# l-johnson-code/glTF-Renderer

Measured on AMD Instinct MI355X. Metric: Mrays/sec + ms/frame @1920x1080, 8-bounce, 1/2/4/8 MI355X, higher is better.
Workload: dtype f32

## Files before the change

### gltf_renderer_amd/csrc/pt_debug_kernels.h

```cpp
#include "pt_vertex.h"
#include "pt_host.h"

namespace pt {
namespace {

__global__ __launch_bounds__(kBlock) void k_debug_sample_texture(SceneRec sc, const uint32_t* __restrict__ mat_slot, const float* __restrict__ tc,
                                                              uint32_t n, float* __restrict__ out, int32_t* __restrict__ taps) {
    stage_luts(sc);
    stage_materials(sc);
    const uint32_t i = blockIdx.x * kBlock + threadIdx.x;
    if (i >= n) return;
    const vec2 uv[2] = {{tc[4 * i], tc[4 * i + 1]}, {tc[4 * i + 2], tc[4 * i + 3]}};
    int32_t t5[5];
    const vec4 r = debug_sample_query(sc, mat_slot[2 * i], (int)mat_slot[2 * i + 1], uv, t5);
    out[4 * i] = r.x; out[4 * i + 1] = r.y; out[4 * i + 2] = r.z; out[4 * i + 3] = r.w;
    for (int c = 0; c < 5; c++) taps[5 * i + c] = t5[c];
}
void launch_debug_sample_texture(const SceneRec& sc, const uint32_t* d_mat_slot, const float* d_tc, uint32_t n, float* d_out, int32_t* d_taps, hipStream_t stream) {
    if (n == 0) return;
    hipLaunchKernelGGL(k_debug_sample_texture, dim3((n + kBlock - 1) / kBlock), dim3(kBlock), 0, stream, sc, d_mat_slot, d_tc, n, d_out, d_taps);
}
__global__ __launch_bounds__(kBlock) void k_debug_env_query(SceneRec sc, int op, const float* __restrict__ in, uint32_t n, float* __restrict__ out) {
#ifdef PT_LUT_LDS
    __shared__ int s_stack[kStackLds * kBlock];
    static_assert((size_t)kStackLds * kBlock * sizeof(int) >= (size_t)kImpLdsFloat4 * sizeof(float4), "the traversal stack's LDS must hold the importance pyramid's coarse levels");
    float4* top = (float4*)s_stack;
    stage_importance_top_into(sc, top);
#else
    const float4* top = importance_lds_top();
#endif
    const uint32_t i = blockIdx.x * kBlock + threadIdx.x;
    if (i >= n) return;
    debug_env_query(sc, op, in + (size_t)kEnvQueryIn * i, out + (size_t)kEnvQueryOut * i, top);
}
void launch_debug_env_query(const SceneRec& sc, int op, const float* d_in, uint32_t n, float* d_out, hipStream_t stream) {
    if (n == 0) return;
    hipLaunchKernelGGL(k_debug_env_query, dim3((n + kBlock - 1) / kBlock), dim3(kBlock), 0, stream, sc, op, d_in, n, d_out);
}
__global__ __launch_bounds__(kBlock) void k_debug_bsdf_query(SceneRec sc, int op, uint32_t flags, const float* __restrict__ in, uint32_t n, float* __restrict__ out) {
    stage_luts(sc);
    const uint32_t i = blockIdx.x * kBlock + threadIdx.x;
    if (i >= n) return;
    debug_bsdf_query(sc, op, flags, in + (size_t)kBsdfQueryIn * i, out + (size_t)kBsdfQueryOut * i);
}
void launch_debug_bsdf_query(const SceneRec& sc, int op, uint32_t flags, const float* d_in, uint32_t n, float* d_out, hipStream_t stream) {
    if (n == 0) return;
    hipLaunchKernelGGL(k_debug_bsdf_query, dim3((n + kBlock - 1) / kBlock), dim3(kBlock), 0, stream, sc, op, flags, d_in, n, d_out);
}
__global__ __launch_bounds__(kBlock) void k_debug_light_query(SceneRec sc_in, uint32_t small_tables, int num_of_lights, const uint32_t* __restrict__ index,
                                                           const float* __restrict__ p, uint32_t n, float* __restrict__ out) {
    SceneRec sc = sc_in; sc.small_tables = small_tables ? 1u : 0u;
    stage_lights(sc, num_of_lights);
    const uint32_t i = blockIdx.x * kBlock + threadIdx.x;
    if (i >= n) return;
    debug_light_query(sc, index[i], v3(p[3 * (size_t)i], p[3 * (size_t)i + 1], p[3 * (size_t)i + 2]), out + (size_t)kLightQueryOut * i);
}
void launch_debug_light_query(const SceneRec& sc, bool small_tables, int num_of_lights, const uint32_t* d_index, const float* d_p, uint32_t n, float* d_out, hipStream_t stream) {
    if (n == 0) return;
    hipLaunchKernelGGL(k_debug_light_query, dim3((n + kBlock - 1) / kBlock), dim3(kBlock), 0, stream, sc, small_tables ? 1u : 0u, num_of_lights, d_index, d_p, n, d_out);
}
__global__ __launch_bounds__(kBlock) void k_debug_surface_query(SceneRec sc_in, uint32_t small_tables, uint32_t flags, const float* __restrict__ in, uint32_t n, float* __restrict__ out) {
    SceneRec sc = sc_in; sc.small_tables = small_tables ? 1u : 0u;
    stage_luts(sc);
    stage_tangent_lut(sc);
    stage_instances(sc);
    stage_materials(sc);
    const uint32_t i = blockIdx.x * kBlock + threadIdx.x;
    if (i >= n) return;
    debug_surface_query(sc, flags, in + (size_t)kSurfQueryIn * i, out + (size_t)kSurfQueryOut * i);
}
void launch_debug_surface_query(const SceneRec& sc, bool small_tables, uint32_t flags, const float* d_in, uint32_t n, float* d_out, hipStream_t stream) {
    if (n == 0) return;
    hipLaunchKernelGGL(k_debug_surface_query, dim3((n + kBlock - 1) / kBlock), dim3(kBlock), 0, stream, sc, small_tables ? 1u : 0u, flags, d_in, n, d_out);
}
constexpr DebugQueryLaunch kDebugQueryLaunch = {launch_debug_sample_texture, launch_debug_env_query, launch_debug_bsdf_query, launch_debug_light_query, launch_debug_surface_query};

// ... 3 lines not shown
```

### gltf_renderer_amd/csrc/pt_shading.h

```cpp
#pragma once
#include "pt_math.h"
#include "pt_types.h"

namespace pt {

constexpr float kMinRoughness = 0.001f;

PT_DEV vec4 next_random(uint32_t px, uint32_t py, uint32_t seed, int& count) {
    uint32_t x = px * 1664525u + 1013904223u, y = py * 1664525u + 1013904223u;
    uint32_t z = seed * 1664525u + 1013904223u, w = (uint32_t)count * 1664525u + 1013904223u;
    count++;
    x += y * w; y += z * x; z += x * y; w += y * z;
    x ^= x >> 16; y ^= y >> 16; z ^= z >> 16; w ^= w >> 16;
    x += y * w; y += z * x; z += x * y; w += y * z;
    const float s = 2.3283064365386963e-10f;
    return {(float)x * s, (float)y * s, (float)z * s, (float)w * s};
}

PT_DEV vec3 decode_octahedral(float ex, float ey) {
    float z = 1.f - fabsf(ex) - fabsf(ey);
    float x = ex, y = ey;
    if (!(z >= 0.f)) {
        x = (ex >= 0 ? 1.f : -1.f) * (1.f - fabsf(ey));
        y = (ey >= 0 ? 1.f : -1.f) * (1.f - fabsf(ex));
// ... 274 lines not shown
    vec3 n, t;
    float tw;
    if (has_ts) {
        vec3 n0, n1, n2, t0, t1, t2;
        float w0, w1, w2;
        decode_tangent_space(ts0, tangent_sincos(sc, (ts0 >> 20) & 0x3ffu), n0, t0, w0);
        decode_tangent_space(ts1, tangent_sincos(sc, (ts1 >> 20) & 0x3ffu), n1, t1, w1);
        decode_tangent_space(ts2, tangent_sincos(sc, (ts2 >> 20) & 0x3ffu), n2, t2, w2);
        n = w.x * n0 + w.y * n1 + w.z * n2;
        t = w.x * t0 + w.y * t1 + w.z * t2;
        tw = w0;
    } else {
        n = ng;
        vec3 helper = v3(1, 0, 0);
        if (fabsf(ng.x) > fabsf(ng.y)) helper = v3(0, 1, 0);
        t = normalize(cross(helper, ng));
        tw = 1;
    }
    a.position = mul_point(in.T, pos);
    a.ng = normalize(mul_dir(in.N, ng));
    a.n = normalize(mul_dir(in.N, n));
    a.t = normalize(mul_dir(in.T, t));
    a.tw = tw;
    a.bt = tw * normalize(cross(a.n, a.t));
    return a;
}

struct Surface {
    vec3 albedo; float alpha, metalness, ax, ay;
    vec3 n, at, ab; float ior;
    vec3 spec_color; float spec_factor, clearcoat, cc_rough;
    vec3 cc_n, sheen_color; float sheen_a, transmissive;
    vec3 emissive_texel;
    float sheen_lh, sheen_sv;
};
struct MatHeader {
    uint32_t flags; int32_t alpha_mode; float metalness_factor, roughness_factor;
    vec4 base_color_factor;
    vec3 emissive_factor; float alpha_cutoff;
    float ior, normal_scale, specular_factor, clearcoat_normal_scale;
    vec3 specular_color_factor; float clearcoat_factor;
    float clearcoat_roughness_factor, anisotropy_strength, anisotropy_cos, anisotropy_sin;
    vec3 sheen_color_factor; float sheen_roughness_factor;
    float transmission_factor; uint32_t bound_mask;
    const uint4* trio;
};
PT_DEV MatHeader load_mat_header(const RMat* m) {
    const float4* q = (const float4*)m;
    const float4 a = q[0], b = q[1], c = q[2], d = q[3], e = q[4], f = q[5], g = q[6], h = q[7];
    MatHeader r;
    r.flags = __float_as_uint(a.x); r.alpha_mode = __float_as_int(a.y); r.metalness_factor = a.z; r.roughness_factor = a.w;
    r.base_color_factor = {b.x, b.y, b.z, b.w};
    r.emissive_factor = v3(c.x, c.y, c.z); r.alpha_cutoff = c.w;
    r.ior = d.x; r.normal_scale = d.y; r.specular_factor = d.z; r.clearcoat_normal_scale = d.w;
    r.specular_color_factor = v3(e.x, e.y, e.z); r.clearcoat_factor = e.w;
    r.clearcoat_roughness_factor = f.x; r.anisotropy_strength = f.y; r.anisotropy_cos = f.z; r.anisotropy_sin = f.w;
    r.sheen_color_factor = v3(g.x, g.y, g.z); r.sheen_roughness_factor = g.w;
    r.transmission_factor = h.x; r.bound_mask = __float_as_uint(h.y);
    r.trio = (const uint4*)(((uint64_t)__float_as_uint(h.w) << 32) | (uint64_t)__float_as_uint(h.z));
    return r;
}
PT_DEV bool slot_bound(uint32_t mask, int slot) { return (mask >> slot) & 1u; }
#ifdef PT_LUT_LDS
constexpr uint32_t kMatCacheMax = 96;
constexpr uint32_t kMatCacheRecs = 17;
static __shared__ float4 pt_lds_mat[kMatCacheMax * kMatCacheRecs];
PT_DEV bool materials_cached(const SceneRec& sc) { return sc.small_tables || sc.n_materials <= kMatCacheMax; }
// ... 182 lines not shown
        const PbrTexels f = fetch_pbr_texels(sc, mid, h, tc);
        const int s = slot == 16 ? SLOT_ALBEDO : slot == 17 ? SLOT_NORMAL : slot == 18 ? SLOT_METALLIC_ROUGHNESS : SLOT_EMISSIVE;
        const bool trio = (h.bound_mask & RM_TRIO) != 0;
        const RTex t = load_rtex(&m->tex[trio ? SLOT_ALBEDO : s]);
        base = t.texels;
        if (slot == 16) { k = f.k_alb; r = resolve_taps(k, f.a00, f.a10, f.a01, f.a11, sc.srgb_lut); }
        else if (slot == 17) { k = f.k_nrm; r = resolve_taps(k, f.n00, f.n10, f.n01, f.n11, sc.srgb_lut); }
        else if (slot == 18) { k = f.k_mr; r = resolve_taps(k, f.m00, f.m10, f.m01, f.m11, sc.srgb_lut); }
        else if (trio && (h.bound_mask & RM_TRIO_EMISSIVE)) { k = f.k_alb; r = f.emissive; }
        else { const RTex te = load_rtex(&m->tex[SLOT_EMISSIVE]); k = texture_taps(te, tc); base = te.texels; r = sample_slot(sc, m, SLOT_EMISSIVE, tc, taps); }
    }
    taps5[0] = k.i0; taps5[1] = k.i1;
    taps5[2] = (int32_t)((k.p0 - base) / k.width); taps5[3] = (int32_t)((k.p1 - base) / k.width);
    taps5[4] = k.ia;
    return r;
}

PT_DEV float schlick(float f0, float c) { return f0 + (1 - f0) * hpow5(1 - fabsf(c)); }
PT_DEV vec3 schlick3(vec3 f0, float c) { return f0 + (1 - f0) * hpow5(1 - fabsf(c)); }
PT_DEV float ggx_d(float a, float ndh) {
    float a2 = a * a;
    float den = ndh * ndh * (a2 - 1) + 1;
    den *= kPi * den;
    return fdiv(a2 * heavyside(ndh), den);
}
PT_DEV float ggx_corr_v(float a, float ndl, float ndv, float hdl, float hdv) {
    float a2 = a * a;
    float num = 0.5f * heavyside(hdl) * heavyside(hdv);
    float den = fabsf(ndv) * sqrtf(a2 + (1 - a2) * ndl * ndl);
    den += fabsf(ndl) * sqrtf(a2 + (1 - a2) * ndv * ndv);
    return fdiv(num, den);
}
PT_DEV float specular_brdf(float a, float ndl, float ndv, float ndh, float hdl, float hdv) { return ggx_corr_v(a, ndl, ndv, hdl, hdv) * ggx_d(a, ndh); }
PT_DEV float ggx_aniso_d(float ax, float ay, vec3 h) {
    float a2 = ax * ay;
    vec3 f = v3(ay * h.x, ax * h.y, a2 * h.z);
    float w2 = fdiv(a2, dot(f, f));
    return fdiv(heavyside(h.z) * a2 * w2 * w2, kPi);
}
PT_DEV float aniso_specular_brdf(float ax, float ay, vec3 v, vec3 h, vec3 l) {
    float hdv = dot(h, v), hdl = dot(h, l);
    float num = 0.5f * heavyside(hdv) * heavyside(hdl);
    float vv = fabsf(l.z) * length(v3(ax * v.x, ay * v.y, v.z));
    float ll = fabsf(v.z) * length(v3(ax * l.x, ay * l.y, l.z));
    return fdiv(num, vv + ll) * ggx_aniso_d(ax, ay, h);
}
PT_DEV float fresnel_coat_w(float weight, float ndv) {
    float f0 = (1 - 1.5f) / (1 + 1.5f);
    f0 *= f0;
    return weight * schlick(f0, ndv);
}
PT_DEV float sheen_l(float alpha, float x) {
    float t = (1 - alpha) * (1 - alpha);
    float a = lerpf(21.5473f, 25.3245f, t), b = lerpf(3.82987f, 3.32435f, t), c = lerpf(0.19823f, 0.16801f, t);
    float d = lerpf(-1.97760f, -1.27393f, t), e = lerpf(-4.32054f, -4.85967f, t);
    return fdiv(a, 1 + b * hpow(x, c)) + d * x + e;
}
PT_DEV float sheen_shadowing(float alpha, float c, float l_half) {
    if (c < 0.5f) return pt_exp(sheen_l(alpha, c));
    return pt_exp(2 * l_half - sheen_l(alpha, 1 - c));
}
PT_DEV float sheen_alpha(const Surface& s) { return clampf(s.sheen_a, 0.000001f, 1); }
PT_DEV void prepare_sheen(Surface& s, vec3 v) {
    const float sa = sheen_alpha(s);
    s.sheen_lh = sheen_l(sa, 0.5f);
    s.sheen_sv = sheen_shadowing(sa, to_local(s.at, s.ab, s.n, v).z, s.sheen_lh);
}
PT_DEV float sheen_brdf(const Surface& s, float alpha, float ndl, float ndv, float ndh) {
    float inv_r = fdiv(1.0f, alpha);
    float sin2h = 1 - ndh * ndh;
    float d = fdiv((2 + inv_r) * hpow(sin2h, inv_r * 0.5f), 2 * kPi);
    float vis = clampf(fdiv(1.0f, (1 + s.sheen_sv + sheen_shadowing(alpha, ndl, s.sheen_lh)) * 4 * ndv * ndl), 0, 1);
    return d * vis;
}
PT_DEV float sheen_e(const float* lut, float alpha, float cos_theta) {
    float x = cos_theta * 16.f - 0.5f, y = alpha * 16.f - 0.5f;
    if (!(x == x)) x = 0;
    if (!(y == y)) y = 0;
    x = clampf(x, -1.f, 16.f); y = clampf(y, -1.f, 16.f);
    float fx0 = floorf(x), fy0 = floorf(y);
    int i0 = (int)fx0, j0 = (int)fy0;
    float fx = x - fx0, fy = y - fy0;
    int ia = max(i0, 0), ib = min(i0 + 1, 15), ja = max(j0, 0), jb = min(j0 + 1, 15);
    ia = min(ia, 15); ja = min(ja, 15); ib = max(ib, 0); jb = max(jb, 0);
    float w00 = (1 - fx) * (1 - fy), w10 = fx * (1 - fy), w01 = (1 - fx) * fy, w11 = fx * fy;
    return sheen_entry(lut, ja * 16 + ia) * w00 + sheen_entry(lut, ja * 16 + ib) * w10 + sheen_entry(lut, jb * 16 + ia) * w01 + sheen_entry(lut, jb * 16 + ib) * w11;
}
PT_DEV float modulate_roughness(float a, float ior) { return clampf(lerpf(0, a, saturate(2 * (ior - 1))), kMinRoughness, 1.0f); }

PT_DEV vec3 gltf_bsdf(const float* lut, const Surface& s, vec3 v, vec3 l, int mode) {
    vec3 n = s.n;
    vec3 h = normalize(v + l);
    vec3 vl = to_local(s.at, s.ab, n, v), hl = to_local(s.at, s.ab, n, h), ll = to_local(s.at, s.ab, n, l);
    float hdl = dot(h, l), hdv = dot(h, v);
    float h_dot_abs_l = dot(normalize(v3(ll.x, ll.y, fabsf(ll.z)) + vl), vl);
    bool refl = mode != 2, trans = mode != 1;
    float cndv = dot(n, v), cndh = dot(n, h), cndl = dot(n, l);
#ifndef PT_PROBE_BASE_ONLY
    const float cc = refl ? saturate(cndl) * specular_brdf(s.cc_rough, cndl, cndv, cndh, hdl, hdv) : 0.f;
#else
    const float cc = 0.f;
#endif
    const float coat_w = fresnel_coat_w(s.clearcoat, cndv);
    float spec = refl ? saturate(ll.z) * aniso_specular_brdf(s.ax, s.ay, vl, hl, ll) : 0.f;
    vec3 diffuse = refl ? saturate(ll.z) * (s.albedo / kPi) : v3(0);
    vec3 transmission = v3(0);
#ifndef PT_PROBE_BASE_ONLY
    if (trans) {
        float a = modulate_roughness(s.ay, s.ior);
        vec3 lr = l - 2 * dot(n, l) * n;
        vec3 hr = normalize(v + lr);
        transmission = saturate(-ll.z) * (s.albedo * specular_brdf(a, dot(n, lr), dot(n, v), dot(n, hr), dot(hr, lr), dot(hr, v)));
    }
#endif
    diffuse = lerp3(diffuse, transmission, s.transmissive);
    float f0s = fdiv(1 - s.ior, 1 + s.ior);
    vec3 f0 = v3(f0s);
    f0 *= f0 * s.spec_color;
    f0 = hmin(f0, v3(1));
    vec3 fr = schlick3(f0, h_dot_abs_l);
    vec3 dielectric = (1 - s.spec_factor * max3(fr)) * diffuse + s.spec_factor * fr * v3(spec);
    vec3 metal = refl ? v3(spec) * schlick3(s.albedo, hdv) : v3(0);
    vec3 material = lerp3(dielectric, metal, s.metalness);
    float sa = sheen_alpha(s);
    float ms = max3(s.sheen_color);
    const bool no_sheen = s.sheen_color.x == 0.0f && s.sheen_color.y == 0.0f && s.sheen_color.z == 0.0f;
    if (!__any(!no_sheen)) {
        const float sin2h = 1 - hl.z * hl.z;
        const float layer = (refl && !(sin2h >= 0.0f)) ? __builtin_nanf("") : 0.0f;
        material = v3(layer) + material * 1.0f;
    } else {
#ifndef PT_PROBE_BASE_ONLY
        vec3 sheen = refl ? v3(saturate(ll.z) * sheen_brdf(s, sa, ll.z, vl.z, hl.z)) : v3(0);
#else
        vec3 sheen = v3(0);
#endif
        float scaling = 1.0f;
        if (ms != 0.0f) scaling = hmin(1.0f - ms * sheen_e(lut, sa, vl.z), 1.0f - ms * sheen_e(lut, sa, ll.z));
        material = s.sheen_color * sheen + material * scaling;
    }
    return lerp3(material, v3(cc), coat_w);
}

PT_DEV vec2 uv_to_square(vec2 uv) { return {uv.x * 2 + -1, uv.y * -2 + 1}; }
PT_DEV vec2 square_to_uv(vec2 s) { return {(s.x - -1) * 0.5f, (s.y - 1) * -0.5f}; }
PT_DEV float square_to_disk_angle(vec2 s, float& r) {
    r = hmax(fabsf(s.x), fabsf(s.y));
    return r == 0 ? 0 : fdiv(kPi * (r + (fabsf(s.y) - fabsf(s.x))), 4 * r);
}
PT_DEV vec2 square_to_disk_finish(vec2 s, float r, float cs, float sn) { return {signf(s.x) * r * cs, signf(s.y) * r * sn}; }
PT_DEV vec2 square_to_disk(vec2 s) {
    float r;
    const float phi = square_to_disk_angle(s, r);
    float sn_, cs_;
    pt_sincos(phi, sn_, cs_);
    return square_to_disk_finish(s, r, cs_, sn_);
}
PT_DEV vec3 square_to_sphere(vec2 s) {
    float d = 1 - (fabsf(s.x) + fabsf(s.y));
    float r = 1 - fabsf(d);
    float phi = (r == 0) ? 0 : (kPi / 4) * (fdiv(fabsf(s.y) - fabsf(s.x), r) + 1);
    float f = r * sqrtf(2 - r * r);
    float sn_, cs_;
    pt_sincos(phi, sn_, cs_);
    return {f * signf(s.x) * cs_, f * signf(s.y) * sn_, signf(d) * (1 - r * r)};
}
PT_DEV vec2 sphere_to_square(vec3 p) {
    float r = sqrtf(1 - fabsf(p.z));
    float phi = pt_atan2(fabsf(p.y), fabsf(p.x));
    float d = signf(p.z) * (1 - r);
    float diff = r * ((4 / kPi) * phi - 1);
// ... 28 lines not shown
    float ct = sqrtf(fdiv(1 - u1, 1 + (a * a - 1) * u1));
    float st = sqrtf(1 - ct * ct);
    return {st * cs, st * sn, ct};
}
PT_DEV vec3 sample_ggx_normal(float a, float u0, float u1) {
    float phi = kTau * u0;
    float sn_, cs_;
    pt_sincos(phi, sn_, cs_);
    return sample_ggx_normal_finish(a, u1, cs_, sn_);
}
PT_DEV float ggx_normal_pdf(float a, vec3 n, vec3 h) { float ndh = dot(n, h); return ggx_d(a, ndh) * ndh; }

struct Lobes { float alpha, clearcoat, sheen, specular, diffuse, transmission; };
PT_DEV Lobes lobe_probabilities(const Surface& s, vec3 v) {
    Lobes p;
    float remaining = 1;
    p.alpha = 1.0f - s.alpha;
    remaining -= p.alpha;
    p.clearcoat = lerpf(0.f, 1.f, fresnel_coat_w(s.clearcoat, dot(s.cc_n, v)));
    p.clearcoat *= remaining;
    remaining -= p.clearcoat;
    p.sheen = any_gt0(s.sheen_color) ? 0.5f : 0.0f;
    p.sheen *= remaining;
    remaining -= p.sheen;
    p.specular = 0.5f;
    p.specular *= remaining;
    remaining -= p.specular;
    p.transmission = s.transmissive;
    p.transmission *= remaining;
    remaining -= p.transmission;
    p.diffuse = remaining;
    return p;
}
PT_DEV float transmission_pdf(const Surface& s, vec3 v, vec3 l) {
    float a = modulate_roughness(s.ay, s.ior);
    l = l - 2 * dot(s.n, l) * s.n;
    vec3 h = normalize(v + l);
    float pdf = ggx_normal_pdf(a, s.n, h);
    pdf = fdiv(pdf, 4 * dot(v, h));
    return pdf;
}
PT_DEV float bsdf_pdf(const Surface& s, vec3 v, vec3 l, bool is_transmission, const Lobes& p) {
    if (is_transmission) return p.transmission * transmission_pdf(s, v, l);
    vec3 h = normalize(v + l);
    float vdh4 = 4 * dot(v, h);
    float cc = ggx_normal_pdf(s.cc_rough, s.cc_n, h);
    cc = fdiv(cc, vdh4);
    float pdf = p.clearcoat * cc;
    float cosp = cosine_hemisphere_pdf(s.n, l);
    pdf += p.sheen * cosp;
    vec3 lh = to_local(s.at, s.ab, s.n, h);
    float sp = ggx_aniso_d(s.ax, s.ay, lh) * lh.z;
    sp = fdiv(sp, vdh4);
    pdf += p.specular * sp;
    pdf += p.diffuse * cosp;
    return pdf;
}
PT_DEV vec3 evaluate_bsdf(uint32_t flags, const float* lut, const Surface& s, const Lobes& p, vec3 ng, vec3 v, vec3 l, float& pdf) {
    if (flags & PT_FLAG_MATERIAL_DIFFUSE_WHITE) {
        float ndl = saturate(dot(s.n, l));
        pdf = fdiv(ndl, kPi);
        return v3(fdiv(ndl, kPi));
    }
    if (flags & PT_FLAG_MATERIAL_MIS) {
        bool is_transmission = (dot(ng, l) * dot(ng, v)) < 0;
        pdf = bsdf_pdf(s, v, l, is_transmission, p);
        return s.alpha * gltf_bsdf(lut, s, v, l, is_transmission ? 2 : 1);
    }
    float ndl = saturate(dot(s.n, l));
    pdf = fdiv(ndl, kPi);
    pdf *= s.alpha;
    return s.alpha * gltf_bsdf(lut, s, v, l, 0);
}
PT_DEV vec3 sample_bsdf(uint32_t flags, const float* lut, const Surface& s, const Lobes& p, vec3 u, vec3 v, vec3& l, float& pdf,
                        bool& is_transmission, bool& use_mis) {
    if (flags & PT_FLAG_MATERIAL_DIFFUSE_WHITE) {
        use_mis = true; is_transmission = false;
        l = sample_cosine_hemisphere(s.n, u.y, u.z);
        pdf = cosine_hemisphere_pdf(s.n, l);
        return v3(fdiv(dot(s.n, l), kPi));
    }
    if (flags & PT_FLAG_MATERIAL_MIS) {
        is_transmission = false; use_mis = true;
        float x = u.x;
        int layer;
        if (x <= p.alpha) layer = 4;
        else { x -= p.alpha;
            if (x <= p.clearcoat) layer = 3;
            else { x -= p.clearcoat;
                if (x <= p.sheen) layer = 2;
                else { x -= p.sheen;
                    if (x <= p.specular) layer = 1;
                    else { x -= p.specular; layer = (x <= p.transmission) ? 5 : 0; } } } }
        if (layer == 4) {
            l = -v; use_mis = false; pdf = p.alpha; is_transmission = true;
            return v3(1 - s.alpha);
        }
        const vec2 sq = uv_to_square({u.y, u.z});
        float disk_r = 0;
        const float disk_phi = square_to_disk_angle(sq, disk_r);
        const float angle = layer == 1 ? disk_phi : kTau * u.y;
        float cs, sn;
        pt_sincos(angle, sn, cs);
        if (layer == 0 || layer == 2) l = sample_cosine_hemisphere_finish(s.n, u.z, cs, sn);
        else if (layer == 1) {
            vec2 d = square_to_disk_finish(sq, disk_r, cs, sn);
            vec3 hl = v3(d.x, d.y, sqrtf(1 - d.x * d.x - d.y * d.y));
            hl.x *= s.ax; hl.y *= s.ay;
            hl = normalize(hl);
            l = reflect(-v, to_world(s.at, s.ab, s.n, hl));
        } else if (layer == 3) {
            vec3 t, b;
            basis_simple(s.cc_n, t, b);
            l = reflect(-v, to_world(t, b, s.cc_n, sample_ggx_normal_finish(s.cc_rough, u.z, cs, sn)));
        } else {
            float a = modulate_roughness(s.ay, s.ior);
            vec3 h = to_world(s.at, s.ab, s.n, sample_ggx_normal_finish(a, u.z, cs, sn));
            l = reflect(-v, h);
            l = l - 2 * dot(s.n, l) * s.n;
            is_transmission = true;
        }
        pdf = bsdf_pdf(s, v, l, is_transmission, p);
        return s.alpha * gltf_bsdf(lut, s, v, l, is_transmission ? 2 : 1);
    }
    if (u.x > s.alpha) {
        l = -v; use_mis = false; pdf = (1 - s.alpha); is_transmission = true;
        return v3(1 - s.alpha);
    }
    use_mis = true; is_transmission = false;
    l = sample_cosine_hemisphere(s.n, u.y, u.z);
    pdf = cosine_hemisphere_pdf(s.n, l);
    pdf *= s.alpha;
    return s.alpha * gltf_bsdf(lut, s, v, l, 0);
}

#ifdef PT_LUT_LDS
constexpr int kLightCacheMax = 32;
static __shared__ float4 pt_lds_light[kLightCacheMax * 4];
PT_DEV void spot_cone_terms(float inner_angle, float outer_angle, float& scale, float& offset) {
    scale = fdiv(1.0f, hmax(0.001f, pt_cos(inner_angle) - pt_cos(outer_angle)));
    offset = -pt_cos(outer_angle) * scale;
}
PT_DEV void stage_lights(const SceneRec& sc, int num_of_lights) {
    const uint32_t n = (uint32_t)(num_of_lights < kLightCacheMax ? num_of_lights : kLightCacheMax), n4 = n * 4u;
    if (threadIdx.x < n4) pt_lds_light[threadIdx.x] = gload_f4((const float4*)sc.lights + threadIdx.x);
    __syncthreads();
    if (threadIdx.x < n) {
        float4& last = pt_lds_light[threadIdx.x * 4u + 3u];
        float scale, offset;
        spot_cone_terms(last.x, last.y, scale, offset);
        last.z = scale; last.w = offset;
    }
    __syncthreads();
}
PT_DEV pt_light load_light(const SceneRec& sc, uint32_t li, bool& cone_terms_staged) {
    float4 q[4];
    cone_terms_staged = sc.small_tables || li < (uint32_t)kLightCacheMax;
    if (cone_terms_staged) { const float4* p = pt_lds_light + li * 4u; q[0] = p[0]; q[1] = p[1]; q[2] = p[2]; q[3] = p[3]; }
    else { const float4* p = (const float4*)sc.lights + (size_t)li * 4u; q[0] = gload_f4(p); q[1] = gload_f4(p + 1); q[2] = gload_f4(p + 2); q[3] = gload_f4(p + 3); }
    pt_light l;
    static_assert(sizeof(pt_light) == 64, "pt_light");
    memcpy(&l, q, 64);
    return l;
}
#else
PT_DEV void spot_cone_terms(float inner_angle, float outer_angle, float& scale, float& offset) {
// ... 179 lines not shown
```

### gltf_renderer_amd/csrc/pt_vertex.h

```cpp
#pragma once
#include "pt_traverse.h"

namespace pt {

struct PathState {
    vec3 beta, thr;
    float prev_pdf;
    int rc, bounce;
    bool prev_mis;
};

struct Followups {
    vec3 add;
    bool overwrite;
    bool q_env, q_light, q_bounce;
    vec3 pend_env, env_dir, pend_light, light_dir, origin_above;
    vec3 b_o, b_d, b_beta, b_thr;
    float b_pdf;
    bool b_mis;
    unsigned counted_shadow;
    uint32_t light_index;
    uint32_t hint_env, hint_light;
};

static_assert(kParkLanes == kBlock, "the parking's rows are one shade workgroup long");
struct ParkRegisters {
    PT_DEV UvInPlace uv(const HitGeom&) const { return UvInPlace(); }
};
struct ParkLds {
    float2* col;
    PT_DEV ParkedUv uv(const HitGeom& va) const {
        col[0] = make_float2(va.tc[0].x, va.tc[0].y); col[kBlock] = make_float2(va.tc[1].x, va.tc[1].y);
        return ParkedUv{col};
    }
};

PT_DEV vec3 miss_environment_color(const SceneRec& sc, float environment_intensity, vec3 dir) {
    return sc.has_env ? environment_intensity * sample_cube(sc.env.cube, sc.env.cube_n, dir) : v3(0);
}
PT_DEV float miss_environment_pdf(const SceneRec& sc, vec3 dir) {
    return sc.has_env ? fdiv(importance_map_pdf(sc.env, square_to_uv(sphere_to_square(normalize(dir)))), 4 * kPi) : 0.f;
}
PT_DEV float miss_mis_weight(float prev_pdf, float env_pdf) { return prev_pdf / (prev_pdf + env_pdf); }

PT_DEV vec3 shade_miss(const SceneRec& sc, const FrameConstants& fc, vec3 dir, const PathState& ps) {
    const uint32_t flags = fc.flags;
    vec3 c;
    if (flags & PT_FLAG_ENVIRONMENT_MAP) {
        c = miss_environment_color(sc, fc.environment_intensity, dir);
        if ((flags & PT_FLAG_ENVIRONMENT_MIS) && ps.prev_mis) c *= miss_mis_weight(ps.prev_pdf, miss_environment_pdf(sc, dir));
    } else c = fc.environment_intensity * v3p(fc.environment_color);
    return ps.beta * c;
}

constexpr int kEnvQueryIn = 8, kEnvQueryOut = 16;
PT_DEV void debug_env_query(const SceneRec& sc, int op, const float* __restrict__ in, float* __restrict__ out, const float4* lds_top) {
    if (op == 0) {
        float pdf;
        uint32_t px, py;
        const vec2 uv = sample_importance_map_texel(sc.env, in[0], in[1], pdf, lds_top, px, py);
        const EnvSample e = environment_light_sample(sc, in[2], in[0], in[1], lds_top);
        out[0] = uv.x; out[1] = uv.y; out[2] = pdf; out[3] = (float)px; out[4] = (float)py;
        out[5] = e.dir.x; out[6] = e.dir.y; out[7] = e.dir.z; out[8] = e.pdf; out[9] = e.color.x; out[10] = e.color.y; out[11] = e.color.z;
    } else if (op == 1) {
        out[0] = importance_map_pdf(sc.env, {in[0], in[1]});
    } else if (op == 2) {
        const vec3 d = {in[0], in[1], in[2]};
        const vec3 c = sample_cube(sc.env.cube, sc.env.cube_n, d);
        out[0] = c.x; out[1] = c.y; out[2] = c.z;
        size_t a[4]; float w[4];
        const bool ok = cube_footprint(sc.env.cube_n, d, a, w);
        const size_t n = (size_t)sc.env.cube_n;
        for (int t = 0; t < 4; t++) {
            out[3 + 3 * t] = ok ? (float)(a[t] / (n * n)) : -1.0f;
            out[4 + 3 * t] = ok ? (float)(a[t] % n) : -1.0f;
            out[5 + 3 * t] = ok ? (float)(a[t] / n % n) : -1.0f;
        }
    } else {
        const vec3 d = {in[0], in[1], in[2]};
        const vec3 c = miss_environment_color(sc, in[4], d);
        const float env_pdf = miss_environment_pdf(sc, d);
        const vec3 m = c * miss_mis_weight(in[3], env_pdf);
        out[0] = c.x; out[1] = c.y; out[2] = c.z; out[3] = env_pdf; out[4] = m.x; out[5] = m.y; out[6] = m.z;
    }
}

PT_DEV Lobes prepare_bsdf(Surface& sp, vec3 view) {
    const Lobes lobes = lobe_probabilities(sp, view);
    sp.sheen_lh = sp.sheen_sv = 0.0f;
    if (__any(sp.sheen_color.x != 0.0f || sp.sheen_color.y != 0.0f || sp.sheen_color.z != 0.0f)) prepare_sheen(sp, view);
    return lobes;
}

constexpr int kBsdfQueryIn = 48, kBsdfQueryOut = 16;
PT_DEV void debug_bsdf_query(const SceneRec& sc, int op, uint32_t flags, const float* __restrict__ in, float* __restrict__ out) {
    Surface sp;
    sp.albedo = v3(in[0], in[1], in[2]); sp.alpha = in[3]; sp.metalness = in[4]; sp.ax = in[5]; sp.ay = in[6];
    sp.n = v3(in[7], in[8], in[9]); sp.at = v3(in[10], in[11], in[12]); sp.ab = v3(in[13], in[14], in[15]); sp.ior = in[16];
    sp.spec_color = v3(in[17], in[18], in[19]); sp.spec_factor = in[20]; sp.clearcoat = in[21]; sp.cc_rough = in[22];
    sp.cc_n = v3(in[23], in[24], in[25]); sp.sheen_color = v3(in[26], in[27], in[28]); sp.sheen_a = in[29]; sp.transmissive = in[30];
    sp.emissive_texel = v3(0);
    const vec3 ng = v3(in[36], in[37], in[38]), view = v3(in[39], in[40], in[41]), a = v3(in[42], in[43], in[44]);
    const Lobes lobes = prepare_bsdf(sp, view);
    vec3 f, l = a;
    float pdf = 0;
    bool is_tr = false, use_mis = false;
    if (op == 0) f = evaluate_bsdf(flags, sc.sheen_e, sp, lobes, ng, view, a, pdf);
    else f = sample_bsdf(flags, sc.sheen_e, sp, lobes, a, view, l, pdf, is_tr, use_mis);
    out[0] = f.x; out[1] = f.y; out[2] = f.z; out[3] = pdf; out[4] = l.x; out[5] = l.y; out[6] = l.z;
    out[7] = is_tr ? 1.0f : 0.0f; out[8] = use_mis ? 1.0f : 0.0f;
    out[9] = lobes.alpha; out[10] = lobes.clearcoat; out[11] = lobes.sheen; out[12] = lobes.specular; out[13] = lobes.diffuse; out[14] = lobes.transmission;
    out[15] = 0.0f;
}
constexpr int kLightQueryOut = 8;
PT_DEV void debug_light_query(const SceneRec& sc, uint32_t li, vec3 p, float* __restrict__ out) {
    vec3 ldir, lcol;
    bool cone_terms_staged;
    const pt_light light = load_light(sc, li, cone_terms_staged);
    light_ray(light, p, ldir, lcol, cone_terms_staged);
    out[0] = ldir.x; out[1] = ldir.y; out[2] = ldir.z; out[3] = lcol.x; out[4] = lcol.y; out[5] = lcol.z;
    out[6] = cone_terms_staged ? 1.0f : 0.0f; out[7] = 0.0f;
}
constexpr int kSurfQueryIn = 8, kSurfQueryOut = 72;
PT_DEV void debug_surface_query(const SceneRec& sc, uint32_t flags, const float* __restrict__ in, float* __restrict__ out) {
    const uint32_t tri = __float_as_uint(in[0]);
    const bool front = __float_as_uint(in[1]) != 0;
    const float hu = in[2], hv = in[3];
    const vec3 d = v3(in[4], in[5], in[6]);
    const ShadePacket* packet_at = sc.shade + tri;
    RawPacket packet = load_shade_packet_raw(packet_at);
    const ShadeInst inst = load_shade_inst(sc, raw_packet_inst(packet));
    if (__any((inst.streams & (SI_TEXCOORD1 | SI_COLOR)) != 0)) {
        if (inst.streams & (SI_TEXCOORD1 | SI_COLOR)) load_shade_packet_extra(packet, packet_at);
    }
    const PacketVerts pv = unpack_shade_packet(packet);
    const RMat* mat = sc.rmats + inst.material_id;
    const MatHeader mh = material_header(sc, inst.material_id);
    HitGeom va = get_vertex_attributes(sc, inst, pv, v3(1 - hu - hv, hu, hv));
    if (!front) { va.ng = -va.ng; va.n = -va.n; va.t = -va.t; va.tw = -va.tw; }
    const vec3 o_above = offset_ray(va.position, va.ng), o_below = offset_ray(va.position, -va.ng);
    const vec3 view = -normalize(d);
// ... 64 lines not shown
        return true;
    }
    if (!hit.front) { va.ng = -va.ng; va.n = -va.n; va.t = -va.t; va.tw = -va.tw; }
    const vec3 intersection = ray.o + (ray.d * hit.t);
    const vec3 o_above = offset_ray(va.position, va.ng), o_below = offset_ray(va.position, -va.ng);
    const vec3 view = -normalize(ray.d);
    const auto uvs = park.uv(va);
    Surface sp = get_surface(sc, flags, mat, mh, va, view, taps, uvs);
    PT_TICK(1)
    if (dbg >= PT_DEBUG_OUTPUT_COLOR && dbg <= PT_DEBUG_OUTPUT_TRANSMISSIVE) {
        vec3 c;
        switch (dbg) {
            case PT_DEBUG_OUTPUT_COLOR: c = sp.albedo; break;
            case PT_DEBUG_OUTPUT_ALPHA: c = v3(sp.alpha); break;
            case PT_DEBUG_OUTPUT_SHADING_NORMAL: c = (sp.n + 1) / 2; break;
            case PT_DEBUG_OUTPUT_SHADING_TANGENT: c = (sp.at + 1) / 2; break;
            case PT_DEBUG_OUTPUT_SHADING_BITANGENT: c = (sp.ab + 1) / 2; break;
            case PT_DEBUG_OUTPUT_METALNESS: c = v3(sp.metalness); break;
            case PT_DEBUG_OUTPUT_ROUGHNESS: c = v3(sqrtf(sp.ay)); break;
            case PT_DEBUG_OUTPUT_SPECULAR: c = v3(sp.spec_factor); break;
            case PT_DEBUG_OUTPUT_SPECULAR_COLOR: c = sp.spec_color; break;
            case PT_DEBUG_OUTPUT_CLEARCOAT: c = v3(sp.clearcoat); break;
            case PT_DEBUG_OUTPUT_CLEARCOAT_ROUGHNESS: c = v3(sp.cc_rough); break;
            case PT_DEBUG_OUTPUT_CLEARCOAT_NORMAL: c = (sp.cc_n + 1) / 2; break;
            default: c = v3(sp.transmissive); break;
        }
        fu.add = ps.beta * c;
        return true;
    }
    if (dbg == PT_DEBUG_OUTPUT_HEMISPHERE_VIEW_SIDE) {
        fu.add = ps.beta * (dot(view, sp.n) > 0 ? v3(0, 1, 0) : v3(1, 0, 0));
        return true;
    }
    const Lobes lobes = lobe_probabilities(sp, view);
    sp.sheen_lh = sp.sheen_sv = 0.0f;
    if (__any(sp.sheen_color.x != 0.0f || sp.sheen_color.y != 0.0f || sp.sheen_color.z != 0.0f)) prepare_sheen(sp, view);
    vec3 c = emissive_of(sc, mat, mh, uvs.of(va), taps, sp.emissive_texel);
    fu.origin_above = o_above;
    PT_TICK(2)
    if (ps.bounce < fc.max_bounces && (flags & PT_FLAG_ENVIRONMENT_MAP) && (flags & PT_FLAG_ENVIRONMENT_MIS)) {
        EnvSample es;
        if (PRE) { es = *pre; ps.rc++; }
        else {
            vec4 r = next_random(px, py, seed, ps.rc);
            es = environment_light_sample(sc, fc.environment_intensity, r.x, r.y, importance_lds_top());
        }
        const float light_pdf = es.pdf;
        const vec3 ldir = es.dir, lcol = es.color;
        PT_TICK(6)
        vec3 contrib = v3(0);
        if (any_gt0(lcol)) {
            float bp = 0;
            vec3 f = evaluate_bsdf(flags, sc.sheen_e, sp, lobes, va.ng, view, ldir, bp);
            float mis = fdiv(light_pdf, light_pdf + bp);
            contrib = (mis * f * lcol) / light_pdf;
        }
        if (flags & PT_FLAG_INDIRECT_ENVIRONMENT_ONLY) c += contrib;
        else {
            fu.pend_env = ps.beta * contrib;
            if (!(fc.cull_null_shadow && fu.pend_env.x == 0.0f && fu.pend_env.y == 0.0f && fu.pend_env.z == 0.0f)) { fu.q_env = true; fu.env_dir = ldir; }
        }
    }
    PT_TICK(3)
    if ((flags & PT_FLAG_POINT_LIGHTS) && fc.num_of_lights > 0) {
        float u = next_random(px, py, seed, ps.rc).x;
        uint32_t li = f2u(u * (float)fc.num_of_lights);
        li = min(li, (uint32_t)(fc.num_of_lights - 1));
        fu.light_index = li;
        float pdf = fdiv(1.0f, (float)fc.num_of_lights);
        vec3 ldir, lcol;
        bool cone_terms_staged;
        const pt_light light = load_light(sc, li, cone_terms_staged);
        light_ray(light, intersection, ldir, lcol, cone_terms_staged);
        vec3 contrib = v3(0);
        if (any_gt0(lcol)) {
            float bp = 0;
            vec3 f = evaluate_bsdf(flags, sc.sheen_e, sp, lobes, va.ng, view, ldir, bp);
            contrib = (lcol * f) / pdf;
        }
        if ((flags & PT_FLAG_SHADOW_RAYS) && !(flags & PT_FLAG_INDIRECT_ENVIRONMENT_ONLY)) {
            fu.pend_light = ps.beta * contrib;
            if (!(fc.cull_null_shadow && fu.pend_light.x == 0.0f && fu.pend_light.y == 0.0f && fu.pend_light.z == 0.0f)) { fu.q_light = true; fu.light_dir = ldir; }
        }
        else c += contrib;
    }
    PT_TICK(4)
    fu.add = ps.beta * c;
    if (ps.bounce < fc.max_bounces) {
        vec4 r = next_random(px, py, seed, ps.rc);
        bool is_tr = false, use_mis = false;
        float bp = 1;
        vec3 l = v3(0);
        vec3 f = sample_bsdf(flags, sc.sheen_e, sp, lobes, v3(r.x, r.y, r.z), view, l, bp, is_tr, use_mis);
        vec3 weight = bp != 0 ? f / bp : v3(0);
        vec3 throughput = ps.thr * weight;
        if (dbg >= PT_DEBUG_OUTPUT_BOUNCE_DIRECTION && dbg <= PT_DEBUG_BOUNCE_IS_TRANSMISSION) {
            vec3 dc;
            switch (dbg) {
                case PT_DEBUG_OUTPUT_BOUNCE_DIRECTION: dc = 0.5f * (l + 1); break;
                case PT_DEBUG_OUTPUT_BOUNCE_BSDF: dc = f; break;
                case PT_DEBUG_OUTPUT_BOUNCE_PDF: dc = v3(bp); break;
                case PT_DEBUG_OUTPUT_BOUNCE_WEIGHT: dc = weight; break;
                default: dc = is_tr ? v3(0, 1, 0) : v3(1, 0, 0); break;
            }
            fu.counted_shadow = (fu.q_env ? 1u : 0u) + (fu.q_light ? 1u : 0u);
            fu.q_env = fu.q_light = false;
            fu.add = ps.beta * dc;
            fu.overwrite = true;
            return true;
        }
        if (any_gt0(throughput)) {
            float ur = next_random(px, py, seed, ps.rc).x;
            bool cont = ps.bounce < fc.min_bounces;
            if (!cont) {
                float p = clampf(max3(throughput), fc.min_rr, fc.max_rr);
                if (ur < p) { weight = weight / p; cont = true; }
            }
            if (cont) {
                fu.q_bounce = true;
                fu.b_o = is_tr ? o_below : o_above;
                fu.b_d = l;
                fu.b_beta = ps.beta * weight;
                fu.b_thr = throughput * weight;
                fu.b_pdf = bp; fu.b_mis = use_mis;
            }
        }
// ... 118 lines not shown
```

Baseline: 6959.

## Hoist view-dependent BSDF terms per vertex and share half-vector work between pdf and eval

Result: faster. 7059, median of 6 (+1.4%).

```diff
diff --git a/gltf_renderer_amd/csrc/pt_debug_kernels.h b/gltf_renderer_amd/csrc/pt_debug_kernels.h
--- a/gltf_renderer_amd/csrc/pt_debug_kernels.h
+++ b/gltf_renderer_amd/csrc/pt_debug_kernels.h
@@ -41,7 +41,11 @@
     stage_luts(sc);
     const uint32_t i = blockIdx.x * kBlock + threadIdx.x;
     if (i >= n) return;
-    debug_bsdf_query(sc, op, flags, in + (size_t)kBsdfQueryIn * i, out + (size_t)kBsdfQueryOut * i);
+#ifdef PT_LUT_LDS
+    debug_bsdf_query<ParkLds>(sc, op, flags, in + (size_t)kBsdfQueryIn * i, out + (size_t)kBsdfQueryOut * i);
+#else
+    debug_bsdf_query<ParkRegisters>(sc, op, flags, in + (size_t)kBsdfQueryIn * i, out + (size_t)kBsdfQueryOut * i);
+#endif
 }
 void launch_debug_bsdf_query(const SceneRec& sc, int op, uint32_t flags, const float* d_in, uint32_t n, float* d_out, hipStream_t stream) {
     if (n == 0) return;
diff --git a/gltf_renderer_amd/csrc/pt_shading.h b/gltf_renderer_amd/csrc/pt_shading.h
--- a/gltf_renderer_amd/csrc/pt_shading.h
+++ b/gltf_renderer_amd/csrc/pt_shading.h
@@ -330,7 +330,16 @@
     vec3 spec_color; float spec_factor, clearcoat, cc_rough;
     vec3 cc_n, sheen_color; float sheen_a, transmissive;
     vec3 emissive_texel;
-    float sheen_lh, sheen_sv;
+};
+struct BsdfView {
+    vec3 vl;
+    float coat_w;
+    vec3 f0;
+    vec3 diffuse;
+    float a2, v_len;
+    float cc_a2, cc_1ma2, cc_sv;
+    float sheen_a, sheen_max, sheen_lh, sheen_sv, sheen_ev;
+    bool no_sheen;
 };
 struct MatHeader {
     uint32_t flags; int32_t alpha_mode; float metalness_factor, roughness_factor;
@@ -579,18 +588,29 @@
     return fdiv(num, den);
 }
 PT_DEV float specular_brdf(float a, float ndl, float ndv, float ndh, float hdl, float hdv) { return ggx_corr_v(a, ndl, ndv, hdl, hdv) * ggx_d(a, ndh); }
-PT_DEV float ggx_aniso_d(float ax, float ay, vec3 h) {
-    float a2 = ax * ay;
+PT_DEV float ggx_d_a2(float a2, float ndh) {
+    float den = ndh * ndh * (a2 - 1) + 1;
+    den *= kPi * den;
+    return fdiv(a2 * heavyside(ndh), den);
+}
+PT_DEV float ggx_corr_v_view(float a2, float one_m_a2, float sv, float ndl, float ndv, float hdl, float hdv) {
+    float num = 0.5f * heavyside(hdl) * heavyside(hdv);
+    float den = fabsf(ndv) * sqrtf(a2 + one_m_a2 * ndl * ndl);
+    den += fabsf(ndl) * sv;
+    return fdiv(num, den);
+}
+PT_DEV float ggx_aniso_d(float ax, float ay, float a2, vec3 h) {
     vec3 f = v3(ay * h.x, ax * h.y, a2 * h.z);
     float w2 = fdiv(a2, dot(f, f));
     return fdiv(heavyside(h.z) * a2 * w2 * w2, kPi);
 }
-PT_DEV float aniso_specular_brdf(float ax, float ay, vec3 v, vec3 h, vec3 l) {
+PT_DEV float aniso_view_length(float ax, float ay, vec3 v) { return length(v3(ax * v.x, ay * v.y, v.z)); }
+PT_DEV float aniso_specular_brdf(float ax, float ay, vec3 v, float v_len, vec3 h, vec3 l, float d) {
     float hdv = dot(h, v), hdl = dot(h, l);
     float num = 0.5f * heavyside(hdv) * heavyside(hdl);
-    float vv = fabsf(l.z) * length(v3(ax * v.x, ay * v.y, v.z));
+    float vv = fabsf(l.z) * v_len;
     float ll = fabsf(v.z) * length(v3(ax * l.x, ay * l.y, l.z));
-    return fdiv(num, vv + ll) * ggx_aniso_d(ax, ay, h);
+    return fdiv(num, vv + ll) * d;
 }
 PT_DEV float fresnel_coat_w(float weight, float ndv) {
     float f0 = (1 - 1.5f) / (1 + 1.5f);
@@ -608,16 +628,11 @@
     return pt_exp(2 * l_half - sheen_l(alpha, 1 - c));
 }
 PT_DEV float sheen_alpha(const Surface& s) { return clampf(s.sheen_a, 0.000001f, 1); }
-PT_DEV void prepare_sheen(Surface& s, vec3 v) {
-    const float sa = sheen_alpha(s);
-    s.sheen_lh = sheen_l(sa, 0.5f);
-    s.sheen_sv = sheen_shadowing(sa, to_local(s.at, s.ab, s.n, v).z, s.sheen_lh);
-}
-PT_DEV float sheen_brdf(const Surface& s, float alpha, float ndl, float ndv, float ndh) {
+PT_DEV float sheen_brdf(float sv, float l_half, float alpha, float ndl, float ndv, float ndh) {
     float inv_r = fdiv(1.0f, alpha);
     float sin2h = 1 - ndh * ndh;
     float d = fdiv((2 + inv_r) * hpow(sin2h, inv_r * 0.5f), 2 * kPi);
-    float vis = clampf(fdiv(1.0f, (1 + s.sheen_sv + sheen_shadowing(alpha, ndl, s.sheen_lh)) * 4 * ndv * ndl), 0, 1);
+    float vis = clampf(fdiv(1.0f, (1 + sv + sheen_shadowing(alpha, ndl, l_half)) * 4 * ndv * ndl), 0, 1);
     return d * vis;
 }
 PT_DEV float sheen_e(const float* lut, float alpha, float cos_theta) {
@@ -635,55 +650,71 @@
 }
 PT_DEV float modulate_roughness(float a, float ior) { return clampf(lerpf(0, a, saturate(2 * (ior - 1))), kMinRoughness, 1.0f); }
 
-PT_DEV vec3 gltf_bsdf(const float* lut, const Surface& s, vec3 v, vec3 l, int mode) {
+struct BsdfHalf {
+    vec3 h, hl;
+    float vdh4, d;
+    float tr_a; vec3 tr_l, tr_h; float tr_ndh, tr_d;
+};
+PT_DEV BsdfHalf half_vectors(const Surface& s, const BsdfView& bv, vec3 v, vec3 l, bool trans) {
+    BsdfHalf k;
+    k.h = normalize(v + l);
+    k.hl = to_local(s.at, s.ab, s.n, k.h);
+    k.vdh4 = 4 * dot(v, k.h);
+    k.d = ggx_aniso_d(s.ax, s.ay, bv.a2, k.hl);
+    k.tr_a = 0; k.tr_l = v3(0); k.tr_h = v3(0); k.tr_ndh = 0; k.tr_d = 0;
+    if (trans) {
+        k.tr_a = modulate_roughness(s.ay, s.ior);
+        k.tr_l = l - 2 * dot(s.n, l) * s.n;
+        k.tr_h = normalize(v + k.tr_l);
+        k.tr_ndh = dot(s.n, k.tr_h);
+        k.tr_d = ggx_d(k.tr_a, k.tr_ndh);
+    }
+    return k;
+}
+
+PT_DEV vec3 gltf_bsdf(const float* lut, const Surface& s, const BsdfView& bv, const BsdfHalf& k, vec3 v, vec3 l, int mode) {
     vec3 n = s.n;
-    vec3 h = normalize(v + l);
-    vec3 vl = to_local(s.at, s.ab, n, v), hl = to_local(s.at, s.ab, n, h), ll = to_local(s.at, s.ab, n, l);
+    vec3 h = k.h;
+    vec3 vl = bv.vl, hl = k.hl, ll = to_local(s.at, s.ab, n, l);
     float hdl = dot(h, l), hdv = dot(h, v);
     float h_dot_abs_l = dot(normalize(v3(ll.x, ll.y, fabsf(ll.z)) + vl), vl);
     bool refl = mode != 2, trans = mode != 1;
-    float cndv = dot(n, v), cndh = dot(n, h), cndl = dot(n, l);
+    float cndv = vl.z, cndh = dot(n, h), cndl = dot(n, l);
 #ifndef PT_PROBE_BASE_ONLY
-    const float cc = refl ? saturate(cndl) * specular_brdf(s.cc_rough, cndl, cndv, cndh, hdl, hdv) : 0.f;
+    const float cc = refl ? saturate(cndl) * (ggx_corr_v_view(bv.cc_a2, bv.cc_1ma2, bv.cc_sv, cndl, cndv, hdl, hdv) * ggx_d_a2(bv.cc_a2, cndh)) : 0.f;
 #else
     const float cc = 0.f;
 #endif
-    const float coat_w = fresnel_coat_w(s.clearcoat, cndv);
-    float spec = refl ? saturate(ll.z) * aniso_specular_brdf(s.ax, s.ay, vl, hl, ll) : 0.f;
-    vec3 diffuse = refl ? saturate(ll.z) * (s.albedo / kPi) : v3(0);
+    const float coat_w = bv.coat_w;
+    float spec = refl ? saturate(ll.z) * aniso_specular_brdf(s.ax, s.ay, vl, bv.v_len, hl, ll, k.d) : 0.f;
+    vec3 diffuse = refl ? saturate(ll.z) * bv.diffuse : v3(0);
     vec3 transmission = v3(0);
 #ifndef PT_PROBE_BASE_ONLY
     if (trans) {
-        float a = modulate_roughness(s.ay, s.ior);
-        vec3 lr = l - 2 * dot(n, l) * n;
-        vec3 hr = normalize(v + lr);
-        transmission = saturate(-ll.z) * (s.albedo * specular_brdf(a, dot(n, lr), dot(n, v), dot(n, hr), dot(hr, lr), dot(hr, v)));
+        const vec3 lr = k.tr_l, hr = k.tr_h;
+        transmission = saturate(-ll.z) * (s.albedo * (ggx_corr_v(k.tr_a, dot(n, lr), vl.z, dot(hr, lr), dot(hr, v)) * k.tr_d));
     }
 #endif
     diffuse = lerp3(diffuse, transmission, s.transmissive);
-    float f0s = fdiv(1 - s.ior, 1 + s.ior);
-    vec3 f0 = v3(f0s);
-    f0 *= f0 * s.spec_color;
-    f0 = hmin(f0, v3(1));
-    vec3 fr = schlick3(f0, h_dot_abs_l);
+    vec3 fr = schlick3(bv.f0, h_dot_abs_l);
     vec3 dielectric = (1 - s.spec_factor * max3(fr)) * diffuse + s.spec_factor * fr * v3(spec);
     vec3 metal = refl ? v3(spec) * schlick3(s.albedo, hdv) : v3(0);
     vec3 material = lerp3(dielectric, metal, s.metalness);
-    float sa = sheen_alpha(s);
-    float ms = max3(s.sheen_color);
-    const bool no_sheen = s.sheen_color.x == 0.0f && s.sheen_color.y == 0.0f && s.sheen_color.z == 0.0f;
+    const float sa = bv.sheen_a;
+    const float ms = bv.sheen_max;
+    const bool no_sheen = bv.no_sheen;
     if (!__any(!no_sheen)) {
         const float sin2h = 1 - hl.z * hl.z;
         const float layer = (refl && !(sin2h >= 0.0f)) ? __builtin_nanf("") : 0.0f;
         material = v3(layer) + material * 1.0f;
     } else {
 #ifndef PT_PROBE_BASE_ONLY
-        vec3 sheen = refl ? v3(saturate(ll.z) * sheen_brdf(s, sa, ll.z, vl.z, hl.z)) : v3(0);
+        vec3 sheen = refl ? v3(saturate(ll.z) * sheen_brdf(bv.sheen_sv, bv.sheen_lh, sa, ll.z, vl.z, hl.z)) : v3(0);
 #else
         vec3 sheen = v3(0);
 #endif
         float scaling = 1.0f;
-        if (ms != 0.0f) scaling = hmin(1.0f - ms * sheen_e(lut, sa, vl.z), 1.0f - ms * sheen_e(lut, sa, ll.z));
+        if (ms != 0.0f) scaling = hmin(1.0f - ms * bv.sheen_ev, 1.0f - ms * sheen_e(lut, sa, ll.z));
         material = s.sheen_color * sheen + material * scaling;
     }
     return lerp3(material, v3(cc), coat_w);
@@ -778,47 +809,96 @@
     p.diffuse = remaining;
     return p;
 }
-PT_DEV float transmission_pdf(const Surface& s, vec3 v, vec3 l) {
-    float a = modulate_roughness(s.ay, s.ior);
-    l = l - 2 * dot(s.n, l) * s.n;
-    vec3 h = normalize(v + l);
-    float pdf = ggx_normal_pdf(a, s.n, h);
-    pdf = fdiv(pdf, 4 * dot(v, h));
+PT_DEV void bsdf_view_terms(const float* lut, const Surface& s, vec3 v, BsdfView& bv) {
+    bv.vl = to_local(s.at, s.ab, s.n, v);
+    bv.coat_w = fresnel_coat_w(s.clearcoat, bv.vl.z);
+    float f0s = fdiv(1 - s.ior, 1 + s.ior);
+    vec3 f0 = v3(f0s);
+    f0 *= f0 * s.spec_color;
+    f0 = hmin(f0, v3(1));
+    bv.f0 = f0;
+    bv.diffuse = s.albedo / kPi;
+    bv.a2 = s.ax * s.ay;
+    bv.v_len = aniso_view_length(s.ax, s.ay, bv.vl);
+    {
+        const float a = s.cc_rough, ndv = bv.vl.z;
+        float a2 = a * a;
+        bv.cc_a2 = a2; bv.cc_1ma2 = 1 - a2;
+        bv.cc_sv = sqrtf(a2 + (1 - a2) * ndv * ndv);
+    }
+    bv.sheen_a = sheen_alpha(s);
+    bv.sheen_max = max3(s.sheen_color);
+    bv.no_sheen = s.sheen_color.x == 0.0f && s.sheen_color.y == 0.0f && s.sheen_color.z == 0.0f;
+    bv.sheen_ev = 0.0f;
+}
+PT_DEV void bsdf_view_sheen_e(const float* lut, BsdfView& bv) {
+    if (bv.sheen_max != 0.0f) bv.sheen_ev = sheen_e(lut, bv.sheen_a, bv.vl.z);
+}
+template <bool VERTEX>
+PT_DEV Lobes prepare_bsdf(const float* lut, const Surface& s, vec3 v, BsdfView& bv) {
+    const Lobes lobes = lobe_probabilities(s, v);
+    if (VERTEX) bsdf_view_terms(lut, s, v, bv);
+    bv.sheen_lh = bv.sheen_sv = 0.0f;
+    if (__any(!(s.sheen_color.x == 0.0f && s.sheen_color.y == 0.0f && s.sheen_color.z == 0.0f))) {
+        const float sa = VERTEX ? bv.sheen_a : sheen_alpha(s);
+        const float ndv = VERTEX ? bv.vl.z : to_local(s.at, s.ab, s.n, v).z;
+        bv.sheen_lh = sheen_l(sa, 0.5f);
+        bv.sheen_sv = sheen_shadowing(sa, ndv, bv.sheen_lh);
+        if (VERTEX) bsdf_view_sheen_e(lut, bv);
+    }
+    return lobes;
+}
+template <bool VERTEX>
+PT_DEV BsdfView view_of(const float* lut, const Surface& s, vec3 v, const BsdfView& prepared) {
+    BsdfView bv = prepared;
+    if (!VERTEX) {
+        bsdf_view_terms(lut, s, v, bv);
+        if (__any(!bv.no_sheen)) bsdf_view_sheen_e(lut, bv);
+    }
+    return bv;
+}
+PT_DEV float transmission_pdf(const BsdfHalf& k, vec3 v) {
+    float pdf = k.tr_d * k.tr_ndh;
+    pdf = fdiv(pdf, 4 * dot(v, k.tr_h));
     return pdf;
 }
-PT_DEV float bsdf_pdf(const Surface& s, vec3 v, vec3 l, bool is_transmission, const Lobes& p) {
-    if (is_transmission) return p.transmission * transmission_pdf(s, v, l);
-    vec3 h = normalize(v + l);
-    float vdh4 = 4 * dot(v, h);
+PT_DEV float bsdf_pdf(const Surface& s, const BsdfHalf& k, vec3 v, vec3 l, bool is_transmission, const Lobes& p) {
+    if (is_transmission) return p.transmission * transmission_pdf(k, v);
+    vec3 h = k.h;
+    float vdh4 = k.vdh4;
     float cc = ggx_normal_pdf(s.cc_rough, s.cc_n, h);
     cc = fdiv(cc, vdh4);
     float pdf = p.clearcoat * cc;
     float cosp = cosine_hemisphere_pdf(s.n, l);
     pdf += p.sheen * cosp;
-    vec3 lh = to_local(s.at, s.ab, s.n, h);
-    float sp = ggx_aniso_d(s.ax, s.ay, lh) * lh.z;
+    vec3 lh = k.hl;
+    float sp = k.d * lh.z;
     sp = fdiv(sp, vdh4);
     pdf += p.specular * sp;
     pdf += p.diffuse * cosp;
     return pdf;
 }
-PT_DEV vec3 evaluate_bsdf(uint32_t flags, const float* lut, const Surface& s, const Lobes& p, vec3 ng, vec3 v, vec3 l, float& pdf) {
+template <bool VERTEX>
+PT_DEV vec3 evaluate_bsdf(uint32_t flags, const float* lut, const Surface& s, const BsdfView& prepared, const Lobes& p, vec3 ng, vec3 v, vec3 l, float& pdf) {
     if (flags & PT_FLAG_MATERIAL_DIFFUSE_WHITE) {
         float ndl = saturate(dot(s.n, l));
         pdf = fdiv(ndl, kPi);
         return v3(fdiv(ndl, kPi));
     }
+    const BsdfView bv = view_of<VERTEX>(lut, s, v, prepared);
     if (flags & PT_FLAG_MATERIAL_MIS) {
         bool is_transmission = (dot(ng, l) * dot(ng, v)) < 0;
-        pdf = bsdf_pdf(s, v, l, is_transmission, p);
-        return s.alpha * gltf_bsdf(lut, s, v, l, is_transmission ? 2 : 1);
+        const BsdfHalf k = half_vectors(s, bv, v, l, is_transmission);
+        pdf = bsdf_pdf(s, k, v, l, is_transmission, p);
+        return s.alpha * gltf_bsdf(lut, s, bv, k, v, l, is_transmission ? 2 : 1);
     }
     float ndl = saturate(dot(s.n, l));
     pdf = fdiv(ndl, kPi);
     pdf *= s.alpha;
-    return s.alpha * gltf_bsdf(lut, s, v, l, 0);
-}
-PT_DEV vec3 sample_bsdf(uint32_t flags, const float* lut, const Surface& s, const Lobes& p, vec3 u, vec3 v, vec3& l, float& pdf,
+    return s.alpha * gltf_bsdf(lut, s, bv, half_vectors(s, bv, v, l, true), v, l, 0);
+}
+template <bool VERTEX>
+PT_DEV vec3 sample_bsdf(uint32_t flags, const float* lut, const Surface& s, const BsdfView& prepared, const Lobes& p, vec3 u, vec3 v, vec3& l, float& pdf,
                         bool& is_transmission, bool& use_mis) {
     if (flags & PT_FLAG_MATERIAL_DIFFUSE_WHITE) {
         use_mis = true; is_transmission = false;
@@ -866,8 +946,10 @@
             l = l - 2 * dot(s.n, l) * s.n;
             is_transmission = true;
         }
-        pdf = bsdf_pdf(s, v, l, is_transmission, p);
-        return s.alpha * gltf_bsdf(lut, s, v, l, is_transmission ? 2 : 1);
+        const BsdfView bv = view_of<VERTEX>(lut, s, v, prepared);
+        const BsdfHalf k = half_vectors(s, bv, v, l, is_transmission);
+        pdf = bsdf_pdf(s, k, v, l, is_transmission, p);
+        return s.alpha * gltf_bsdf(lut, s, bv, k, v, l, is_transmission ? 2 : 1);
     }
     if (u.x > s.alpha) {
         l = -v; use_mis = false; pdf = (1 - s.alpha); is_transmission = true;
@@ -877,7 +959,8 @@
     l = sample_cosine_hemisphere(s.n, u.y, u.z);
     pdf = cosine_hemisphere_pdf(s.n, l);
     pdf *= s.alpha;
-    return s.alpha * gltf_bsdf(lut, s, v, l, 0);
+    const BsdfView bv = view_of<VERTEX>(lut, s, v, prepared);
+    return s.alpha * gltf_bsdf(lut, s, bv, half_vectors(s, bv, v, l, true), v, l, 0);
 }
 
 #ifdef PT_LUT_LDS
diff --git a/gltf_renderer_amd/csrc/pt_vertex.h b/gltf_renderer_amd/csrc/pt_vertex.h
--- a/gltf_renderer_amd/csrc/pt_vertex.h
+++ b/gltf_renderer_amd/csrc/pt_vertex.h
@@ -25,9 +25,11 @@
 
 static_assert(kParkLanes == kBlock, "the parking's rows are one shade workgroup long");
 struct ParkRegisters {
+    static constexpr bool kBsdfViewPerVertex = false;
     PT_DEV UvInPlace uv(const HitGeom&) const { return UvInPlace(); }
 };
 struct ParkLds {
+    static constexpr bool kBsdfViewPerVertex = true;
     float2* col;
     PT_DEV ParkedUv uv(const HitGeom& va) const {
         col[0] = make_float2(va.tc[0].x, va.tc[0].y); col[kBlock] = make_float2(va.tc[1].x, va.tc[1].y);
@@ -85,14 +87,8 @@
     }
 }
 
-PT_DEV Lobes prepare_bsdf(Surface& sp, vec3 view) {
-    const Lobes lobes = lobe_probabilities(sp, view);
-    sp.sheen_lh = sp.sheen_sv = 0.0f;
-    if (__any(sp.sheen_color.x != 0.0f || sp.sheen_color.y != 0.0f || sp.sheen_color.z != 0.0f)) prepare_sheen(sp, view);
-    return lobes;
-}
-
 constexpr int kBsdfQueryIn = 48, kBsdfQueryOut = 16;
+template <class Park>
 PT_DEV void debug_bsdf_query(const SceneRec& sc, int op, uint32_t flags, const float* __restrict__ in, float* __restrict__ out) {
     Surface sp;
     sp.albedo = v3(in[0], in[1], in[2]); sp.alpha = in[3]; sp.metalness = in[4]; sp.ax = in[5]; sp.ay = in[6];
@@ -101,12 +97,14 @@
     sp.cc_n = v3(in[23], in[24], in[25]); sp.sheen_color = v3(in[26], in[27], in[28]); sp.sheen_a = in[29]; sp.transmissive = in[30];
     sp.emissive_texel = v3(0);
     const vec3 ng = v3(in[36], in[37], in[38]), view = v3(in[39], in[40], in[41]), a = v3(in[42], in[43], in[44]);
-    const Lobes lobes = prepare_bsdf(sp, view);
+    constexpr bool kVertex = Park::kBsdfViewPerVertex;
+    BsdfView bv;
+    const Lobes lobes = prepare_bsdf<kVertex>(sc.sheen_e, sp, view, bv);
     vec3 f, l = a;
     float pdf = 0;
     bool is_tr = false, use_mis = false;
-    if (op == 0) f = evaluate_bsdf(flags, sc.sheen_e, sp, lobes, ng, view, a, pdf);
-    else f = sample_bsdf(flags, sc.sheen_e, sp, lobes, a, view, l, pdf, is_tr, use_mis);
+    if (op == 0) f = evaluate_bsdf<kVertex>(flags, sc.sheen_e, sp, bv, lobes, ng, view, a, pdf);
+    else f = sample_bsdf<kVertex>(flags, sc.sheen_e, sp, bv, lobes, a, view, l, pdf, is_tr, use_mis);
     out[0] = f.x; out[1] = f.y; out[2] = f.z; out[3] = pdf; out[4] = l.x; out[5] = l.y; out[6] = l.z;
     out[7] = is_tr ? 1.0f : 0.0f; out[8] = use_mis ? 1.0f : 0.0f;
     out[9] = lobes.alpha; out[10] = lobes.clearcoat; out[11] = lobes.sheen; out[12] = lobes.specular; out[13] = lobes.diffuse; out[14] = lobes.transmission;
@@ -237,9 +235,9 @@
         fu.add = ps.beta * (dot(view, sp.n) > 0 ? v3(0, 1, 0) : v3(1, 0, 0));
         return true;
     }
-    const Lobes lobes = lobe_probabilities(sp, view);
-    sp.sheen_lh = sp.sheen_sv = 0.0f;
-    if (__any(sp.sheen_color.x != 0.0f || sp.sheen_color.y != 0.0f || sp.sheen_color.z != 0.0f)) prepare_sheen(sp, view);
+    constexpr bool kVertex = Park::kBsdfViewPerVertex;
+    BsdfView bv;
+    const Lobes lobes = prepare_bsdf<kVertex>(sc.sheen_e, sp, view, bv);
     vec3 c = emissive_of(sc, mat, mh, uvs.of(va), taps, sp.emissive_texel);
     fu.origin_above = o_above;
     PT_TICK(2)
@@ -256,7 +254,7 @@
         vec3 contrib = v3(0);
         if (any_gt0(lcol)) {
             float bp = 0;
-            vec3 f = evaluate_bsdf(flags, sc.sheen_e, sp, lobes, va.ng, view, ldir, bp);
+            vec3 f = evaluate_bsdf<kVertex>(flags, sc.sheen_e, sp, bv, lobes, va.ng, view, ldir, bp);
             float mis = fdiv(light_pdf, light_pdf + bp);
             contrib = (mis * f * lcol) / light_pdf;
         }
@@ -280,7 +278,7 @@
         vec3 contrib = v3(0);
         if (any_gt0(lcol)) {
             float bp = 0;
-            vec3 f = evaluate_bsdf(flags, sc.sheen_e, sp, lobes, va.ng, view, ldir, bp);
+            vec3 f = evaluate_bsdf<kVertex>(flags, sc.sheen_e, sp, bv, lobes, va.ng, view, ldir, bp);
             contrib = (lcol * f) / pdf;
         }
         if ((flags & PT_FLAG_SHADOW_RAYS) && !(flags & PT_FLAG_INDIRECT_ENVIRONMENT_ONLY)) {
@@ -296,7 +294,7 @@
         bool is_tr = false, use_mis = false;
         float bp = 1;
         vec3 l = v3(0);
-        vec3 f = sample_bsdf(flags, sc.sheen_e, sp, lobes, v3(r.x, r.y, r.z), view, l, bp, is_tr, use_mis);
+        vec3 f = sample_bsdf<kVertex>(flags, sc.sheen_e, sp, bv, lobes, v3(r.x, r.y, r.z), view, l, bp, is_tr, use_mis);
         vec3 weight = bp != 0 ? f / bp : v3(0);
         vec3 throughput = ps.thr * weight;
         if (dbg >= PT_DEBUG_OUTPUT_BOUNCE_DIRECTION && dbg <= PT_DEBUG_BOUNCE_IS_TRANSMISSION) {
```
